# HyTruongSon/GraphFlow

Hardware: AMD Instinct MI355X
Metric: CCN-2D (SMP_omega) molecules/sec fwd+bwd (higher is better)
Workload: dtype f32 (level block products: 2xf16-split operands, 22-bit, fp32 accumulate); 1 GPU; cfg3: SMP_omega 3 levels, C=64, F=5, D=5, cap=29, batch=1024 synthetic QM9-size molecules/GPU, device-resident, fused levels; parallelism=single GPU

## Files before the change

### graphflow_amd/csrc/smp_fused.hip

```cpp
#include <algorithm>
#include <type_traits>

#include "r18_device.h"
#include "smp_internal.h"

using namespace gf::dev;

namespace gf {
namespace {

__device__ __forceinline__ f4 fold_two_tables(f4 u, f4 v) {
    f4 z;
#pragma unroll
    for (int k = 0; k < 4; ++k) {
        const auto r = __builtin_amdgcn_permlane16_swap(__float_as_uint(u[k]), __float_as_uint(v[k]), false, false);
        z[k] = xor32_sum(__uint_as_float(r[0]) + __uint_as_float(r[1]));
    }
    return z;
}

__device__ __forceinline__ f4 dpp_xor8(f4 v) {
    f4 r;
#pragma unroll
    for (int k = 0; k < 4; ++k)
        r[k] = __int_as_float(__builtin_amdgcn_update_dpp(0, __float_as_int(v[k]), 0x128 , 0xf, 0xf, true));
    return r;
}

__device__ __forceinline__ f4 dpp_ror4(f4 v) {
    f4 r;
#pragma unroll
    for (int k = 0; k < 4; ++k)
        r[k] = __int_as_float(__builtin_amdgcn_update_dpp(0, __float_as_int(v[k]), 0x124 , 0xf, 0xf, true));
    return r;
}

constexpr float kAlphaF = 0.01f;
__device__ __forceinline__ float lreluf(float z) { return z > 0.f ? z : kAlphaF * z; }

enum { T_SAB = 0, T_SBC = 1, T_T6 = 2, T_T10 = 3, T_COLS = 4 };
enum { O_LOC = 0, O_Z = 1, O_ZP = 2, O_COLS = 3 };
__constant__ int c_kperm[18] = {0, 2, 6, 5, 9, 8, 12, 11, 15, 16, 1, 3, 7, 10, 4, 13, 14, 17};

#ifndef GF_TF_DEPTH2
#define GF_TF_DEPTH2 0
#endif
#ifndef GF_TF_OCC
#define GF_TF_OCC 4
#endif
#ifndef GF_TF_WIDE
#define GF_TF_WIDE 16
#endif
#ifndef GF_TF_D2NI
#define GF_TF_D2NI 4
#endif
template <int NI, bool ALLOK, bool VEC = false, int LPC = 16>
__global__ __launch_bounds__(NI >= GF_TF_WIDE ? 2 * kThreads : kThreads, NI <= 4 ? GF_TF_OCC : 2) void smp_tables_fwd_w(
    const float *__restrict__ fprev, const float *__restrict__ rsum,
                                                             float *__restrict__ T, float *__restrict__ Vt,
                                                             float *__restrict__ scal, const long long *__restrict__ pair_src_row,
                                                             const int *__restrict__ pair_src_s, const short *__restrict__ pi,
                                                             const int4 *__restrict__ recs,
                                                             int C, int nwin,
                                                             int zeros_kept,
                                                             const unsigned char *__restrict__ rowflag,
                                                             float *__restrict__ St) {
    static_assert(!VEC || ALLOK, "the folded vector sums need every lane to have channels");
    constexpr int PPW = 64 / LPC, CWIN = 4 * LPC;
    static_assert(LPC == 16 || ((LPC == 8 || LPC == 4) && ALLOK), "eight / four lanes per position: whole 32- / 16-channel windows only");
    const int tid = threadIdx.x, lane = tid & 63;
    const int wave = __builtin_amdgcn_readfirstlane(tid >> 6);
    const int cg = lane / LPC, fl = lane % LPC;
    unsigned tile;
    {
        const unsigned nb = gridDim.x, qq = nb / 8, r = nb % 8, x = blockIdx.x % 8;
        tile = (x < r ? x * (qq + 1) : r * (qq + 1) + (x - r) * qq) + blockIdx.x / 8;
    }
    const int win = (int)(tile % nwin);
    const int4 r0 = recs[2 * (tile / nwin)], r1 = recs[2 * (tile / nwin) + 1];
    const int N = r0.y;
    const size_t rowbase = ((size_t)(unsigned)r1.y << 32) | (unsigned)r1.x, pairbase = ((size_t)(unsigned)r1.w << 32) | (unsigned)r1.z;
    const int f = win * CWIN + 4 * fl;
    const bool fok = f < C;
    const int fld = fok ? f : 0;
    constexpr bool allok = ALLOK;

    extern __shared__ __attribute__((aligned(16))) float smem[];
    constexpr int ST = PPW * NI;
    constexpr int kAbsent = 0x40000000;
    float *sR = smem;
    int4 *sRow = reinterpret_cast<int4 *>(smem + ((N + 3) & ~3));
    int *sOff = reinterpret_cast<int *>(sRow + N);
    const int nthreads = (NI >= GF_TF_WIDE ? 2 : 1) * kThreads;
    for (int i = tid; i < N; i += nthreads) {
        sR[i] = rsum[pairbase + i];
        const int sw = pair_src_s[pairbase + i];
        const unsigned long long addr = reinterpret_cast<unsigned long long>(fprev + pair_src_row[pairbase + i] * C);
        sRow[i] = make_int4((int)(unsigned)addr, (int)(unsigned)(addr >> 32), sw * sw * C * 4, sw);
    }
    for (int i = tid; i < N * ST; i += nthreads) {
        const int a = i / ST, c = i % ST;
        const int p = (c < N) ? pi[rowbase + a * N + c] : -1;
        sOff[i] = p >= 0 ? p * C * 4 : kAbsent;
    }
    unsigned char *sFlag = reinterpret_cast<unsigned char *>(sOff + N * ST);
    const bool skip_bc = zeros_kept && rowflag;
    if (skip_bc)
        for (int i = tid; i < N * N; i += nthreads) sFlag[i] = rowflag[rowbase + i];
    f4 *sAcc = reinterpret_cast<f4 *>(smem + ((((N + 3) & ~3) + 4 * N + N * ST + ((N * N + 3) >> 2) + 3) & ~3));
    const int nwv = nthreads / 64;
    f4 *wacc = sAcc + (size_t)wave * N * (2 * LPC), *wdummy = sAcc + (size_t)nwv * N * (2 * LPC) + wave * (2 * LPC);
    if constexpr (VEC)
        for (int i = lane; i < N * (2 * LPC); i += 64) wacc[i] = splat(0.f);
    __syncthreads();

    float rc[NI];
    int cc[NI];
#pragma unroll
    for (int i = 0; i < NI; ++i) {
        const int c = i * PPW + cg;
        cc[i] = (c < N) ? c : -1;
        rc[i] = (c < N && fok) ? sR[c] : 0.f;
    }
    for (int b = wave; b < N; b += nthreads / 64) {
    f4 sbc[NI], t10[NI];
#pragma unroll
    for (int i = 0; i < NI; ++i) sbc[i] = t10[i] = splat(0.f);
    f4 dgsum = splat(0.f);

    const int lane_off = fok ? fld * 4 : kAbsent;
    const int diag_off = (cg < 2) ? lane_off : kAbsent;
    auto load_row = [&](int a, f4(&v)[NI], f4 &dg) {
        const int4 ri = sRow[a];
        const int *orow = sOff + a * ST;
        const int ob = orow[b];
        int oc[NI];
#pragma unroll
        for (int i = 0; i < NI; ++i) oc[i] = orow[cg + PPW * i];
        const int od = orow[(cg == 0) ? b : a];
        const unsigned lo = __builtin_amdgcn_readfirstlane((unsigned)ri.x), hi = __builtin_amdgcn_readfirstlane((unsigned)ri.y);
        const int bytes = __builtin_amdgcn_readfirstlane(ri.z), sw = __builtin_amdgcn_readfirstlane(ri.w);
        const float *src = reinterpret_cast<const float *>(((unsigned long long)hi << 32) | lo);
        const __amdgpu_buffer_rsrc_t rs = make_rsrc(src, (size_t)(unsigned)bytes);
        const int rowoff = __builtin_amdgcn_readfirstlane(ob) * sw;
#pragma unroll
        for (int i = 0; i < NI; ++i) v[i] = buf_ld4(rs, oc[i] + lane_off, rowoff);
        dg = buf_ld4(rs, od + diag_off, rowoff);
    };

    f4 bufA[NI], bufB[NI], dA, dB;
    float *const tcol = T + (rowbase + b) * (size_t)(T_COLS * C) + f + (((lane >> 4) & 1) ? T_T6 : T_SAB) * C;
    const size_t tstep = (size_t)N * (T_COLS * C);
    unsigned present = (unsigned)__ballot(lane < N && sOff[(lane < N ? lane : 0) * ST + b] != kAbsent);
    present = __builtin_amdgcn_readfirstlane(present);
    if (allok) {
        if (!zeros_kept)
            for (unsigned z = ~present & (N >= 32 ? 0xffffffffu : ((1u << N) - 1u)); z; z &= z - 1)
                st4(tcol + (__builtin_ctz(z)) * tstep, splat(0.f));
    } else if (fok && cg < 2) {
        for (unsigned z = ~present & (N >= 32 ? 0xffffffffu : ((1u << N) - 1u)); z; z &= z - 1)
            st4(T + (rowbase + (size_t)__builtin_ctz(z) * N + b) * (size_t)(T_COLS * C) + f + (cg ? T_T6 : T_SAB) * C, splat(0.f));
    }
    auto row_step = [&](int a, int an, const f4(&cur)[NI], const f4 &dcur, f4(&nxt)[NI], f4 &dnxt, auto own_row) {
        load_row(an >= 0 ? an : a, nxt, dnxt);
        const float ra = sR[a];
        f4 sab = splat(0.f), t6 = splat(0.f);
#pragma unroll
        for (int i = 0; i < NI; ++i) {
            const f4 v = cur[i];
            sbc[i] += v;
            t10[i] += ra * v;
            sab += v;
            t6 += rc[i] * v;
        }
        if constexpr (LPC <= 8) {
            sab += dpp_xor8(sab);
            t6 += dpp_xor8(t6);
        }
        if constexpr (LPC == 4) {
            sab += dpp_ror4(sab);
            t6 += dpp_ror4(t6);
        }
        const f4 both = fold_two_tables(sab, t6);
        dgsum += dcur;
        if (allok) {
            gf_st_s<32>(reinterpret_cast<f4 *>(tcol + a * tstep), both);
            if constexpr (VEC) {
                f4 *slot = (cg == 0) ? wacc + a * (2 * LPC) + fl : wdummy + fl;
                const f4 r = slot[0] + both, d8 = slot[LPC] + dcur;
                slot[0] = r;
                slot[LPC] = d8;
            }
            if constexpr (decltype(own_row)::value) {
                if (cg == 0) st4(scal + ((pairbase + b) * 4 + 3) * (size_t)C + f, dcur);
                if (cg == 2 * (16 / LPC)) st4(scal + ((pairbase + b) * 4 + 1) * (size_t)C + f, both);
            }
        } else if (fok) {
            float *trow = T + (rowbase + (size_t)a * N + b) * (size_t)(T_COLS * C) + f;
            if (cg == 0) {
                st4(trow + T_SAB * C, both);
                if (a == b) st4(scal + ((pairbase + b) * 4 + 3) * (size_t)C + f, dcur);
            } else if (cg == 1) {
                st4(trow + T_T6 * C, both);
            } else if (cg == 2) {
                if (a == b) st4(scal + ((pairbase + b) * 4 + 1) * (size_t)C + f, both);
            }
        }
    };
    {
        auto pop = [&]() {
            if (!present) return -1;
            const int a = __builtin_ctz(present);
            present &= present - 1;
            return a;
        };
        if (ALLOK) {
            present &= ~(1u << b);
            if constexpr (GF_TF_DEPTH2 && NI <= GF_TF_D2NI) {
                f4 bufC[NI], dC;
                int a1 = pop(), a2 = pop();
                load_row(b, bufA, dA);
                load_row(a1 >= 0 ? a1 : b, bufB, dB);
                row_step(b, a2, bufA, dA, bufC, dC, std::true_type{});
                while (a1 >= 0) {
                    const int a3 = pop();
                    row_step(a1, a3, bufB, dB, bufA, dA, std::false_type{});
                    if (a2 < 0) break;
                    const int a4 = pop();
                    row_step(a2, a4, bufC, dC, bufB, dB, std::false_type{});
                    if (a3 < 0) break;
                    const int a5 = pop();
                    row_step(a3, a5, bufA, dA, bufC, dC, std::false_type{});
                    a1 = a4;
                    a2 = a5;
                }
            } else {
            int a = b, an = pop();
            load_row(a, bufA, dA);
            row_step(a, an, bufA, dA, bufB, dB, std::true_type{});
            while (an >= 0) {
                a = an;
                an = pop();
                row_step(a, an, bufB, dB, bufA, dA, std::false_type{});
                if (an < 0) break;
                a = an;
                an = pop();
                row_step(a, an, bufA, dA, bufB, dB, std::false_type{});
            }
            }
        } else {
            int a = pop();
            load_row(a, bufA, dA);
            for (;;) {
                int an = pop();
                row_step(a, an, bufA, dA, bufB, dB, std::false_type{});
                if (an < 0) break;
                a = an;
                an = pop();
                row_step(a, an, bufB, dB, bufA, dA, std::false_type{});
                if (an < 0) break;
                a = an;
            }
        }
    }
    f4 cs = splat(0.f);
#pragma unroll
    for (int i = 0; i < NI; ++i) {
        if (cc[i] >= 0) {
            cs += sbc[i];
            if (fok && (!skip_bc || (sFlag[b * N + cc[i]] & 2))) {
                float *trow = T + (rowbase + (size_t)b * N + cc[i]) * (size_t)(T_COLS * C) + f;
                gf_st_s<32>(reinterpret_cast<f4 *>(trow + T_SBC * C), sbc[i]);
                gf_st_s<32>(reinterpret_cast<f4 *>(trow + T_T10 * C), t10[i]);
            }
        }
    }
    cs = reduce_cgroups<LPC>(cs);
    const f4 dactot = shfl_xor4(dgsum, LPC);
    if (cg == 0 && fok) {
        float *v = Vt + (pairbase + b) * 4 * (size_t)C + f;
        st4(v + 1 * C, cs);
        st4(v + 3 * C, dactot);
        float *sc = scal + (pairbase + b) * 4 * (size_t)C + f;
        st4(sc + 0 * C, cs);
        st4(sc + 2 * C, dgsum);
    }
    }
    if constexpr (VEC) {
        __syncthreads();
        const int node = r0.x;
        for (int i = tid; i < N * (2 * LPC); i += nthreads) {
            const int a = i / (2 * LPC), rem = i % (2 * LPC);
            f4 v = sAcc[(size_t)a * (2 * LPC) + rem];
            for (int w = 1; w < nwv; ++w) v += sAcc[((size_t)w * N + a) * (2 * LPC) + rem];
            st4(Vt + (pairbase + a) * 4 * (size_t)C + (rem / LPC) * 2 * C + win * CWIN + 4 * (rem % LPC), v);
        }
        if (tid < 4 * LPC) {
            const int k = tid / LPC, q = tid % LPC;
            const auto one = [](int) { return 1.f; };
            st4(St + (size_t)node * 4 * C + k * C + win * CWIN + 4 * q,
                batched_sum(scal + pairbase * 4 * (size_t)C + k * C + win * CWIN + 4 * q, (size_t)4 * C, 0, N, one));
        }
    }
}

constexpr int kBigN = 64;
__global__ __launch_bounds__(256) void smp_tables_fwd_big(const float *__restrict__ fprev, const float *__restrict__ rsum, float *__restrict__ T,
                                                          float *__restrict__ Vt, float *__restrict__ scal,
                                                          const long long *__restrict__ pair_src_row, const int *__restrict__ pair_src_s,
                                                          const short *__restrict__ pi, const int *__restrict__ pair_node,
                                                          const int *__restrict__ node_s, const long long *__restrict__ node_row,
                                                          const long long *__restrict__ node_pair, long long pair0, int C, int zeros_kept,
                                                          const unsigned char *__restrict__ rowflag) {
    const long long e = pair0 + blockIdx.x;
    const int n = pair_node[e], N = node_s[n];
    const size_t rowbase = (size_t)node_row[n], pairbase = (size_t)node_pair[n];
    const int b = (int)(e - (long long)pairbase), nl = C >> 2, tid = threadIdx.x;
    extern __shared__ __attribute__((aligned(16))) float big_smem[];
    float *sBC = big_smem;
    float *sAC = sBC + (size_t)N * C;
    float *sR = sAC + (size_t)N * C;
    long long *sSrc = reinterpret_cast<long long *>(sR + ((N + 3) & ~3));
    int *sSw = reinterpret_cast<int *>(sSrc + N);
    short *sPi = reinterpret_cast<short *>(sSw + N);
    for (int i = tid; i < N; i += 256) {
        sR[i] = rsum[pairbase + i];
        sSrc[i] = pair_src_row[pairbase + i] * C;
        sSw[i] = pair_src_s[pairbase + i];
    }
    for (int i = tid; i < N * N; i += 256) sPi[i] = pi[rowbase + i];
    __syncthreads();
    const bool skip_bc = zeros_kept && rowflag;
    for (int it = tid; it < N * nl; it += 256) {
        const int c = it / nl, f = 4 * (it - c * nl);
        f4 sbc = splat(0.f), t10 = splat(0.f);
        for (int a = 0; a < N; ++a) {
            const int pb = sPi[a * N + b], pc = sPi[a * N + c];
            if (pb >= 0 && pc >= 0) {
                const f4 v = ld4(fprev + sSrc[a] + ((size_t)pb * sSw[a] + pc) * C + f);
                sbc += v;
                t10 += sR[a] * v;
            }
        }
        st4(sBC + (size_t)c * C + f, sbc);
        if (!skip_bc || (rowflag[rowbase + (size_t)b * N + c] & 2)) {
            float *trow = T + (rowbase + (size_t)b * N + c) * (size_t)(T_COLS * C) + f;
            st4(trow + T_SBC * C, sbc);
            st4(trow + T_T10 * C, t10);
        }
    }
    __syncthreads();
    f4 cs = splat(0.f);
    if (tid < nl)
        for (int c = 0; c < N; ++c) cs += ld4(sBC + (size_t)c * C + 4 * tid);
    __syncthreads();
    for (int it = tid; it < N * nl; it += 256) {
        const int a = it / nl, f = 4 * (it - a * nl);
        const int pb = sPi[a * N + b];
        f4 sab = splat(0.f), t6 = splat(0.f), dbb = splat(0.f), dac = splat(0.f);
        if (pb >= 0) {
            const float *src = fprev + sSrc[a] + (size_t)pb * sSw[a] * C + f;
            for (int c = 0; c < N; ++c) {
                const int pc = sPi[a * N + c];
                if (pc >= 0) {
                    const f4 v = ld4(src + (size_t)pc * C);
                    sab += v;
                    t6 += sR[c] * v;
                    if (c == b) dbb = v;
                    if (c == a) dac = v;
                }
            }
        }
        if (pb >= 0 || !zeros_kept) {
            float *trow = T + (rowbase + (size_t)a * N + b) * (size_t)(T_COLS * C) + f;
            st4(trow + T_SAB * C, sab);
            st4(trow + T_T6 * C, t6);
        }
        st4(sBC + (size_t)a * C + f, dbb);
        st4(sAC + (size_t)a * C + f, dac);
        if (a == b) {
            st4(scal + ((pairbase + b) * 4 + 3) * (size_t)C + f, dbb);
            st4(scal + ((pairbase + b) * 4 + 1) * (size_t)C + f, sab);
        }
    }
    __syncthreads();
    if (tid < nl) {
        const int f = 4 * tid;
        f4 dgsum = splat(0.f), dactot = splat(0.f);
        for (int a = 0; a < N; ++a) {
            dgsum += ld4(sBC + (size_t)a * C + f);
            dactot += ld4(sAC + (size_t)a * C + f);
        }
        float *v = Vt + (pairbase + b) * 4 * (size_t)C + f;
        st4(v + 1 * C, cs);
        st4(v + 3 * C, dactot);
        float *sc = scal + (pairbase + b) * 4 * (size_t)C + f;
        st4(sc + 0 * C, cs);
        st4(sc + 2 * C, dgsum);
    }
}
static size_t tables_big_lds(int N, int C) {
    return sizeof(float) * (2 * (size_t)N * C + ((N + 3) & ~3)) + sizeof(long long) * N + sizeof(int) * N + sizeof(short) * (size_t)N * N + 32;
}

__global__ __launch_bounds__(256) void smp_vectors(const float *__restrict__ T, float *__restrict__ Vt,
                                                   const float *__restrict__ scal, float *__restrict__ St,
                                                   const int *__restrict__ node_s, const long long *__restrict__ node_row,
                                                   const long long *__restrict__ node_pair, int C,
                                                   const float *__restrict__ Fdc, const long long *__restrict__ pair_src_pair,
                                                   const short *__restrict__ pi) {
    const int n = blockIdx.x;
    const int s = node_s[n], nl = C / 4;
    const size_t rowbase = (size_t)node_row[n], pairbase = (size_t)node_pair[n];
    const auto one = [](int) { return 1.f; };
    for (int i = threadIdx.x; i < s * nl; i += blockDim.x) {
        const int fl = i % nl, x = i / nl;
        const float *t = T + (rowbase + (size_t)x * s) * (size_t)(T_COLS * C) + T_SAB * C + 4 * fl;
        f4 rs = splat(0.f), d8 = splat(0.f);
        {
            const float *fd = Fdc + (size_t)pair_src_pair[pairbase + x] * 2 * C + 4 * fl;
            const short *map = pi + rowbase + (size_t)x * s;
            for (int b0 = 0; b0 < s; b0 += 8) {
                f4 v[8], u[8];
                bool ok[8];
#pragma unroll
                for (int j = 0; j < 8; ++j) {
                    const int p = (b0 + j < s) ? map[b0 + j] : -1;
                    ok[j] = p >= 0;
                    v[j] = ld4(fd + (size_t)(ok[j] ? p : 0) * 2 * C);
                    u[j] = ld4(ok[j] ? t + (size_t)(b0 + j) * (T_COLS * C) : fd);
                }
#pragma unroll
                for (int j = 0; j < 8; ++j)
                    if (ok[j]) d8 += v[j], rs += u[j];
            }
        }
        st4(Vt + (pairbase + x) * 4 * (size_t)C + 0 * C + 4 * fl, rs);
        st4(Vt + (pairbase + x) * 4 * (size_t)C + 2 * C + 4 * fl, d8);
    }
    for (int i = threadIdx.x; i < C; i += blockDim.x)
        st4(St + (size_t)n * 4 * C + 4 * i, batched_sum(scal + pairbase * 4 * (size_t)C + 4 * i, (size_t)4 * C, 0, s, one));
}

__global__ void diag_gather_fwd(const float *__restrict__ fprev, float *__restrict__ Fdc, const int *__restrict__ node_s,
                                const long long *__restrict__ node_row, const long long *__restrict__ node_pair,
                                const int *__restrict__ node_center, int C) {
    const int w = blockIdx.x;
    const int s = node_s[w], c = node_center[w], nl = C / 4;
    const float *src = fprev + (size_t)node_row[w] * C;
    float *dst = Fdc + (size_t)node_pair[w] * 2 * C;
    for (int i = threadIdx.x; i < s * nl; i += blockDim.x) {
        const int fl = i % nl, p = i / nl;
        st4(dst + (size_t)p * 2 * C + 4 * fl, ld4(src + ((size_t)p * s + p) * C + 4 * fl));
        st4(dst + (size_t)p * 2 * C + C + 4 * fl, ld4(src + ((size_t)p * s + c) * C + 4 * fl));
    }
}
// ... 433 lines not shown
    bool live[NI];
#pragma unroll
    for (int i = 0; i < NI; ++i) {
        const int c = i * PPW + cg;
        const bool ok = c < N;
        const int cx = ok ? c : 0;
        cxs[i] = cx;
        live[i] = ok && fok;
        coff[i] = cx * C + fc;
        rc[i] = L.r[cx];
        const float *t = dT + (rowbase + (size_t)b * N + cx) * (size_t)(T_COLS * C) + fc;
        yv[i] = ld4(t + T_SBC * C);
        g9[i] = ld4(t + T_T10 * C);
    }
    const int ib = b / PPW, cgb = b % PPW;
    float *dPg = dP + pbase * C + (size_t)b * N * C;
    const size_t rowStride = (size_t)N * N * C;
    for (int a = wave; a < N; a += kWaves) {
        const short *map = sPi + a * N;
        if (map[b] < 0) continue;
        float *row = dPg + a * rowStride;
        const f4 xa = ld4(sX + a * CW + 4 * fl), g5a = ld4(sG5 + a * CW + 4 * fl);
        const float ra = L.r[a];
        const int ia = a / PPW, cga = a % PPW;
        const f4 z1 = ld4(sZ1 + a * CW + 4 * fl) * ((cg == cgb) ? 1.f : 0.f);
        const f4 z2 = ld4(sZ2 + a * CW + 4 * fl) * ((cg == cga) ? 1.f : 0.f);
#pragma unroll
        for (int i = 0; i < NI; ++i) {
            f4 o = xa + yv[i] + g5a * rc[i] + g9[i] * ra;
            if (i == ib) o += z1;
            if (i == ia) o += z2;
            if (live[i] && map[cxs[i]] >= 0) st4(row + coff[i], o);
        }
    }
}

template <int LPC>
size_t tables_bwd_lds(int N) {
    constexpr int CW = 4 * LPC;
    return sizeof(float) * ((size_t)adj_lds_floats(N) + 4 * (size_t)N * CW) + sizeof(short) * (size_t)N * N + 16;
}
template <int LPC>
size_t combine_lds(int N) {
    constexpr int CW = 4 * LPC;
    return sizeof(float) * ((size_t)adj_lds_floats(N) + (size_t)kCombX * (N + 1) * CW);
}

static int node_block(const gfsmp::LevelLayout &h, int C) {
    const int smax = h.buckets.empty() ? 1 : h.buckets.back().s;
    int t = (smax * (C / 4) + 63) / 64 * 64;
    return t < 64 ? 64 : t > 256 ? 256 : t;
}

struct SizeClass {
    long long lo, hi;
    int smax, ni;
};

std::vector<SizeClass> classes_of(const gfsmp::LevelLayout &h, int ppw) {
    std::vector<SizeClass> out;
    size_t k = 0;
    for (int cls = 1; cls <= 8 && k < h.buckets.size(); cls *= 2) {
        const size_t k0 = k;
        int smax = 0;
        while (k < h.buckets.size() && h.buckets[k].s <= cls * ppw && h.buckets[k].s <= 32) smax = h.buckets[k++].s;
        if (k == k0) continue;
        SizeClass c;
        c.lo = h.node_pair[h.buckets[k0].first_node];
        c.hi = (k < h.buckets.size()) ? h.node_pair[h.buckets[k].first_node] : (long long)h.pairs;
        c.smax = smax;
        c.ni = cls;
        out.push_back(c);
    }
    return out;
}

struct BigPart {
    int n0 = 0, nodes = 0, quad0 = 0, quads = 0, smax = 0;
    long long row0 = 0, pair0 = 0, pairs = 0;
};
static BigPart big_part(const gfsmp::LevelLayout &h) {
    BigPart b;
    b.n0 = h.nNodes, b.row0 = h.rows, b.pair0 = h.pairs, b.quad0 = (int)h.quad_node.size();
    long long q = 0;
    for (const gfsmp::Bucket &bk : h.buckets) {
        if (bk.s > 32) {
            b.n0 = bk.first_node;
            break;
        }
        q += (long long)bk.count * ((bk.s + 3) / 4);
    }
    if (b.n0 < h.nNodes) {
        b.nodes = h.nNodes - b.n0;
        b.row0 = h.node_row[(size_t)b.n0], b.pair0 = h.node_pair[(size_t)b.n0];
        b.pairs = h.pairs - b.pair0;
        b.quad0 = (int)q, b.quads = (int)h.quad_node.size() - (int)q;
        b.smax = h.buckets.back().s;
    }
    return b;
}

Ragged ragged_for(const gf_smp::DevLevel &d, long long lo, int smax) {
    Ragged R = {d.pair_node, d.node_s, d.node_p, d.node_row, d.node_pair, lo, smax};
    return R;
}

static bool smp_half_window(int C) { return C % 32 == 0 && C % 64 != 0; }
static bool smp_quarter_window(int C) { return C == 16; }

static bool smp_tables_fold_vectors(const gf_smp *s) {
    return (s->cfg.nChanels & 63) == 0 || smp_half_window(s->cfg.nChanels) || smp_quarter_window(s->cfg.nChanels);
}

template <int NI>
constexpr const char *tables_fwd_name() {
    return NI == 1 ? "smpf_tables_fwd_ni1" : NI == 2 ? "smpf_tables_fwd_ni2" : NI == 4 ? "smpf_tables_fwd_ni4" : "smpf_tables_fwd_ni8";
}
template <int NI, int LPC>
gf_status launch_tables_fwd_wn(gf_smp *s, int l, const SizeClass &c) {
    gf_ctx *ctx = s->ctx;
    const gf_smp::DevLevel &d = s->lv[l];
    const gfsmp::LevelLayout &h = s->lay.level[l];
    const int C = s->cfg.nChanels, nwin = C / (4 * LPC);
    constexpr int PPW = 64 / LPC;
    const int n_lo = h.pair_node[(size_t)c.lo], n_hi = (c.hi < (long long)h.pairs) ? h.pair_node[(size_t)c.hi] : h.nNodes;
    if (n_hi <= n_lo) return GF_OK;
    const size_t lds = sizeof(float) * ((c.smax + 3) & ~3) + 16 * (size_t)c.smax + sizeof(int) * (size_t)c.smax * PPW * NI + 16 +
                       (size_t)c.smax * c.smax + 16;
    const int nwv = kThreads / 64;
    const size_t lds_v = ((lds + 15) & ~(size_t)15) + 16 + (size_t)nwv * ((size_t)c.smax * (32 * LPC) + 32 * LPC);
    gf_status st = opt_in_lds(ctx, smp_tables_fwd_w<NI, true, true, LPC>, lds_v);
    if (st != GF_OK) return st;
    const int flags = d.t_zeros ? 1 : 0;
    GF_LAUNCH(ctx, tables_fwd_name<NI>(), (smp_tables_fwd_w<NI, true, true, LPC>), dim3((unsigned)((n_hi - n_lo) * nwin)), dim3(kThreads), lds_v,
              s->lv[l - 1].f, d.rsum, d.Q, d.Vt, d.scal, d.pair_src_row, d.pair_src_s, d.pi, d.tf_recs + 2 * (size_t)n_lo, C, nwin,
              flags, flags ? d.rowflag : (const unsigned char *)nullptr, d.St);
    return GF_OK;
}

template <int NI>
gf_status launch_tables_fwd_w(gf_smp *s, int l, const SizeClass &c) {
    gf_ctx *ctx = s->ctx;
    const gf_smp::DevLevel &d = s->lv[l];
    const gfsmp::LevelLayout &h = s->lay.level[l];
    const int C = s->cfg.nChanels, nwin = (C + 63) / 64;
    const int n_lo = h.pair_node[(size_t)c.lo], n_hi = (c.hi < (long long)h.pairs) ? h.pair_node[(size_t)c.hi] : h.nNodes;
    if (n_hi <= n_lo) return GF_OK;
    const size_t lds = sizeof(float) * ((c.smax + 3) & ~3) + 16 * (size_t)c.smax + sizeof(int) * (size_t)c.smax * 4 * NI + 16 +
                       (size_t)c.smax * c.smax + 16;
    const int flags = ((d.t_zeros && (C & 63) == 0) ? 1 : 0);
    if (smp_tables_fold_vectors(s)) {
        const int nwv = (NI >= GF_TF_WIDE ? 2 : 1) * kThreads / 64;
        const size_t lds_v = ((lds + 15) & ~(size_t)15) + 16 + (size_t)nwv * ((size_t)c.smax * 512 + 512);
        gf_status st = opt_in_lds(ctx, smp_tables_fwd_w<NI, true, true>, lds_v);
        if (st != GF_OK) return st;
        GF_LAUNCH(ctx, tables_fwd_name<NI>(), (smp_tables_fwd_w<NI, true, true>), dim3((unsigned)((n_hi - n_lo) * nwin)), dim3((NI >= GF_TF_WIDE ? 2 : 1) * kThreads), lds_v,
                  s->lv[l - 1].f, d.rsum, d.Q, d.Vt, d.scal, d.pair_src_row, d.pair_src_s, d.pi, d.tf_recs + 2 * (size_t)n_lo, C, nwin,
                  flags, flags ? d.rowflag : (const unsigned char *)nullptr, d.St);
    } else
        GF_LAUNCH(ctx, tables_fwd_name<NI>(), (smp_tables_fwd_w<NI, false>), dim3((unsigned)((n_hi - n_lo) * nwin)), dim3((NI >= GF_TF_WIDE ? 2 : 1) * kThreads), lds,
                  s->lv[l - 1].f, d.rsum, d.Q, d.Vt, d.scal, d.pair_src_row, d.pair_src_s, d.pi, d.tf_recs + 2 * (size_t)n_lo, C, nwin,
                  flags, (const unsigned char *)nullptr, (float *)nullptr);
    return GF_OK;
}

template <int NI>
gf_status launch_tables_bwd(gf_smp *s, int l, const SizeClass &c, const float *dT) {
    gf_ctx *ctx = s->ctx;
    const gf_smp::DevLevel &d = s->lv[l];
    const int C = s->cfg.nChanels, nwin = (C + 63) / 64;
    const size_t lds = tables_bwd_lds<16>(c.smax);
    gf_status st = opt_in_lds(ctx, smp_tables_bwd<16, NI>, lds);
    if (st != GF_OK) return st;
    GF_LAUNCH(ctx, "smpf_tables_bwd", (smp_tables_bwd<16, NI>), dim3((unsigned)((c.hi - c.lo) * nwin)), dim3(kThreads), lds, dT,
              d.dVt, d.dSt, d.adj, s->P, d.pi, ragged_for(d, c.lo, c.smax), C, nwin);
    return GF_OK;
}


constexpr int kGatherMaxS = 64;

struct GatherTables {
    const int4 *hdr;
    const int4 *qrec;
};

__global__ __launch_bounds__(64) void build_gather_records(const int *__restrict__ prev_s, const long long *__restrict__ cons_ptr,
                                     const long long *__restrict__ cons_qbase, const int *__restrict__ cons_s,
                                     const int *__restrict__ cons_a, const long long *__restrict__ cons_row,
                                     const long long *__restrict__ cons_pair, const int *__restrict__ pair_node,
                                     const long long *__restrict__ cons_inv_off, const short *__restrict__ inv,
                                     const float *__restrict__ rsum, int ldt_bytes, int4 *__restrict__ hdr, int4 *__restrict__ qrec) {
    const int w = blockIdx.x, sw = prev_s[w];
    const int pad = gfsmp::gather_pad(sw);
    const long long c0 = cons_ptr[w], c1 = cons_ptr[w + 1], qb = cons_qbase[w];
    for (long long ce = c0 + threadIdx.x; ce < c1; ce += blockDim.x) {
        const long long row = cons_row[ce], pe = cons_pair[ce], pb = pe - cons_a[ce];
        hdr[2 * ce] = make_int4(cons_s[ce], cons_a[ce], (int)(unsigned)(row & 0xffffffffll), (int)(row >> 32));
        hdr[2 * ce + 1] = make_int4((int)(unsigned)(pb & 0xffffffffll), (int)(pb >> 32), pair_node[pe], __float_as_int(rsum[pe]));
    }
    const long long n = (c1 - c0) * pad;
    for (long long i = threadIdx.x; i < n; i += blockDim.x) {
        const long long ce = c0 + i / pad;
        const int q = (int)(i % pad);
        const long long pe = cons_pair[ce], pb = pe - cons_a[ce];
        const int c = q < sw ? (int)inv[cons_inv_off[ce] + q] : -1;
        int cfirst = 0;
        for (int k = 0; k < sw; ++k) {
            const int ck = (int)inv[cons_inv_off[ce] + k];
            if (ck >= 0) {
                cfirst = ck;
                break;
            }
        }
        const float ra = rsum[pe], rho = c >= 0 ? rsum[pb + c] : 0.f, m = c >= 0 ? 1.f : 0.f;
        qrec[qb + i] = make_int4((c >= 0 ? c : cfirst) * ldt_bytes, __float_as_int(rho), __float_as_int(m), __float_as_int(m * ra));
    }
}

typedef int si4 __attribute__((ext_vector_type(4)));
__device__ __forceinline__ si4 s_load4(const int4 *p) {
    si4 r;
    asm volatile("s_load_dwordx4 %0, %1, 0x0" : "=s"(r) : "s"(p));
    return r;
}
__device__ __forceinline__ void s_wait2(si4 &a, si4 &b) { asm volatile("s_waitcnt lgkmcnt(0)" : "+s"(a), "+s"(b)); }
template <int N>
__device__ __forceinline__ void s_wait(si4 (&r)[N]) {
    if constexpr (N == 1) asm volatile("s_waitcnt lgkmcnt(0)" : "+s"(r[0]));
    else if constexpr (N == 2) asm volatile("s_waitcnt lgkmcnt(0)" : "+s"(r[0]), "+s"(r[1]));
    else if constexpr (N == 4) asm volatile("s_waitcnt lgkmcnt(0)" : "+s"(r[0]), "+s"(r[1]), "+s"(r[2]), "+s"(r[3]));
    else if constexpr (N == 5) asm volatile("s_waitcnt lgkmcnt(0)" : "+s"(r[0]), "+s"(r[1]), "+s"(r[2]), "+s"(r[3]), "+s"(r[4]));
    else if constexpr (N == 6)
        asm volatile("s_waitcnt lgkmcnt(0)" : "+s"(r[0]), "+s"(r[1]), "+s"(r[2]), "+s"(r[3]), "+s"(r[4]), "+s"(r[5]));
    else {
        static_assert(N == 8, "batch sizes of the gather");
        asm volatile("s_waitcnt lgkmcnt(0)"
                     : "+s"(r[0]), "+s"(r[1]), "+s"(r[2]), "+s"(r[3]), "+s"(r[4]), "+s"(r[5]), "+s"(r[6]), "+s"(r[7]));
    }
}

__device__ __forceinline__ f4 gbuf_ld4_once(__amdgpu_buffer_rsrc_t r, int voff_bytes) {
    return __builtin_bit_cast(f4, __builtin_amdgcn_raw_buffer_load_b128(r, voff_bytes, 0, (GF_NT_SITES & 128) ? 2 : 0));
}
constexpr int kOor = 0x40000000;

#define GF_GATHER_PARAMS                                                                                                          \
    const float *__restrict__ dT, const float *__restrict__ dVt, const float *__restrict__ dSt, float *__restrict__ dfprev,            \
        const float *__restrict__ dFdc, const int *__restrict__ prev_s, const long long *__restrict__ prev_row,                      \
        const long long *__restrict__ prev_pair, const int *__restrict__ prev_center, const long long *__restrict__ cons_ptr,        \
        const long long *__restrict__ cons_inv_off, const long long *__restrict__ cons_qbase, const short *__restrict__ inv,         \
        GatherTables G, int C
#define GF_GATHER_ARGS dT, dVt, dSt, dfprev, dFdc, prev_s, prev_row, prev_pair, prev_center, cons_ptr, cons_inv_off, cons_qbase, inv, G, C

template <int SWP, int QB, int RS = SWP>
__device__ __forceinline__ void gather_source(GF_GATHER_PARAMS, int w, int chunk, int qoff = 0) {
    static_assert(SWP % QB == 0, "whole batches");
    const int sw = prev_s[w], cw = prev_center[w];
    const int nl = C >> 2, items = sw * nl;
    const long long c0 = cons_ptr[w], c1 = cons_ptr[w + 1];
    const int C4 = C * 4, ldtb = T_COLS * C4;
    float *dst = dfprev + prev_row[w] * C;
    const float *dfd = dFdc + (size_t)prev_pair[w] * 2 * C;
    const long long ioff0 = c0 < c1 ? cons_inv_off[c0] : 0;
    const int4 *qr0 = G.qrec + cons_qbase[w];
    {
        const int it = chunk * 64 + (int)(threadIdx.x & 63);
        const bool live = it < items;
        const int p = live ? it / nl : 0, f4b = 16 * (live ? it % nl : 0);
        f4 acc[SWP], accd = splat(0.f), accc = splat(0.f);
#pragma unroll
        for (int q = 0; q < SWP; ++q) acc[q] = splat(0.f);
        if (live) {
            accd = ld4(dfd + (size_t)p * 2 * C + (f4b >> 2));
            accc = ld4(dfd + (size_t)p * 2 * C + C + (f4b >> 2));
        }
        if (c0 < c1) {
            si4 h0 = s_load4(G.hdr + 2 * c0), h1 = s_load4(G.hdr + 2 * c0 + 1);
            s_wait2(h0, h1);
            int b = inv[ioff0 + p];
            b = live ? b : -1;
            for (long long ce = c0; ce < c1; ++ce) {
                const long long cn = ce + 1 < c1 ? ce + 1 : ce;
                si4 n0 = s_load4(G.hdr + 2 * cn), n1 = s_load4(G.hdr + 2 * cn + 1);
                int bn = inv[ioff0 + (cn - c0) * sw + p];
                bn = live ? bn : -1;
                const int s = h0.x, a = h0.y;
                const long long urow = ((long long)h0.w << 32) | (unsigned)h0.z, upb = ((long long)h1.y << 32) | (unsigned)h1.x;
                const int unode = h1.z;
                const __amdgpu_buffer_rsrc_t rT = make_rsrc(dT + (size_t)urow * (T_COLS * C), (size_t)s * s * ldtb);
                const __amdgpu_buffer_rsrc_t rV = make_rsrc(dVt + (size_t)upb * 4 * C, (size_t)s * 4 * C4);
                const __amdgpu_buffer_rsrc_t rS = make_rsrc(dSt + (size_t)unode * 4 * C, (size_t)4 * C4);
                const bool has = b >= 0;
                const int tab = has ? (a * s + b) * ldtb + f4b : kOor;
                const int va = has ? a * 4 * C4 + f4b : kOor, vb = has ? b * 4 * C4 + f4b : kOor;
                const int vs = has ? f4b : kOor, vd = (has && p == cw) ? f4b : kOor;
                const int tb = has ? b * s * ldtb + f4b : kOor;
                const f4 l0 = gbuf_ld4_once(rT, tab + T_SAB * C4), g5 = gbuf_ld4_once(rT, tab + T_T6 * C4);
                const f4 l1 = buf_ld4(rV, va, 0), l4 = buf_ld4(rV, va + 2 * C4, 0);
                const f4 l2 = buf_ld4(rV, vb + C4, 0), z2 = buf_ld4(rV, vb + 3 * C4, 0);
                const f4 l3 = buf_ld4(rS, vs, 0), l5 = buf_ld4(rS, vs + 2 * C4, 0);
                const f4 l6 = buf_ld4(rS, vd + C4, 0), l7 = buf_ld4(rS, vd + 3 * C4, 0);
                const int4 *qr = qr0 + (ce - c0) * RS + qoff;
                f4 x = splat(0.f);
#pragma unroll
                for (int q0 = 0; q0 < SWP; q0 += QB) {
// ... 700 lines not shown
```

Before: 164,100 molecules/s.

## Dispatch forward table kernel to exact-width NI instantiation per node size

Moves the forward table-building body into a device function and adds a multi-width kernel that picks, per node, the template instantiation whose position count NI is just large enough for that node's size, through a wave-uniform switch. A size class no longer pays for the worst-case NI registers and loop trips on smaller nodes. It also rebuilds the per-slot column index inside the store loop instead of keeping it in a register array, to ease register pressure. In exchange the kernel grows in code size and may need more registers, since one kernel holds several inlined bodies. It is on by default for NI 4 and 8 when vector folding is enabled, and an environment variable turns it off.

```diff
diff --git a/graphflow_amd/csrc/smp_fused.hip b/graphflow_amd/csrc/smp_fused.hip
--- a/graphflow_amd/csrc/smp_fused.hip
+++ b/graphflow_amd/csrc/smp_fused.hip
@@ -54,30 +54,21 @@
 #ifndef GF_TF_D2NI
 #define GF_TF_D2NI 4
 #endif
-template <int NI, bool ALLOK, bool VEC = false, int LPC = 16>
-__global__ __launch_bounds__(NI >= GF_TF_WIDE ? 2 * kThreads : kThreads, NI <= 4 ? GF_TF_OCC : 2) void smp_tables_fwd_w(
-    const float *__restrict__ fprev, const float *__restrict__ rsum,
-                                                             float *__restrict__ T, float *__restrict__ Vt,
-                                                             float *__restrict__ scal, const long long *__restrict__ pair_src_row,
-                                                             const int *__restrict__ pair_src_s, const short *__restrict__ pi,
-                                                             const int4 *__restrict__ recs,
-                                                             int C, int nwin,
-                                                             int zeros_kept,
-                                                             const unsigned char *__restrict__ rowflag,
-                                                             float *__restrict__ St) {
+template <int NI, bool ALLOK, bool VEC, int LPC>
+__device__ __forceinline__ void tables_fwd_node(const float *__restrict__ fprev, const float *__restrict__ rsum, float *__restrict__ T,
+                                                float *__restrict__ Vt, float *__restrict__ scal, const long long *__restrict__ pair_src_row,
+                                                const int *__restrict__ pair_src_s, const short *__restrict__ pi,
+                                                const int4 r0, const int4 r1,
+                                                const int win, int C,
+                                                int zeros_kept,
+                                                const unsigned char *__restrict__ rowflag,
+                                                float *__restrict__ St) {
     static_assert(!VEC || ALLOK, "the folded vector sums need every lane to have channels");
     constexpr int PPW = 64 / LPC, CWIN = 4 * LPC;
     static_assert(LPC == 16 || ((LPC == 8 || LPC == 4) && ALLOK), "eight / four lanes per position: whole 32- / 16-channel windows only");
     const int tid = threadIdx.x, lane = tid & 63;
     const int wave = __builtin_amdgcn_readfirstlane(tid >> 6);
     const int cg = lane / LPC, fl = lane % LPC;
-    unsigned tile;
-    {
-        const unsigned nb = gridDim.x, qq = nb / 8, r = nb % 8, x = blockIdx.x % 8;
-        tile = (x < r ? x * (qq + 1) : r * (qq + 1) + (x - r) * qq) + blockIdx.x / 8;
-    }
-    const int win = (int)(tile % nwin);
-    const int4 r0 = recs[2 * (tile / nwin)], r1 = recs[2 * (tile / nwin) + 1];
     const int N = r0.y;
     const size_t rowbase = ((size_t)(unsigned)r1.y << 32) | (unsigned)r1.x, pairbase = ((size_t)(unsigned)r1.w << 32) | (unsigned)r1.z;
     const int f = win * CWIN + 4 * fl;
@@ -115,11 +106,9 @@
     __syncthreads();
 
     float rc[NI];
-    int cc[NI];
 #pragma unroll
     for (int i = 0; i < NI; ++i) {
         const int c = i * PPW + cg;
-        cc[i] = (c < N) ? c : -1;
         rc[i] = (c < N && fok) ? sR[c] : 0.f;
     }
     for (int b = wave; b < N; b += nthreads / 64) {
@@ -264,12 +253,15 @@
         }
     }
     f4 cs = splat(0.f);
+    int cg_b = cg;
+    asm volatile("" : "+v"(cg_b));
 #pragma unroll
     for (int i = 0; i < NI; ++i) {
-        if (cc[i] >= 0) {
+        const int c = i * PPW + cg_b;
+        if (c < N) {
             cs += sbc[i];
-            if (fok && (!skip_bc || (sFlag[b * N + cc[i]] & 2))) {
-                float *trow = T + (rowbase + (size_t)b * N + cc[i]) * (size_t)(T_COLS * C) + f;
+            if (fok && (!skip_bc || (sFlag[b * N + c] & 2))) {
+                float *trow = T + (rowbase + (size_t)b * N + c) * (size_t)(T_COLS * C) + f;
                 gf_st_s<32>(reinterpret_cast<f4 *>(trow + T_SBC * C), sbc[i]);
                 gf_st_s<32>(reinterpret_cast<f4 *>(trow + T_T10 * C), t10[i]);
             }
@@ -302,6 +294,44 @@
                 batched_sum(scal + pairbase * 4 * (size_t)C + k * C + win * CWIN + 4 * q, (size_t)4 * C, 0, N, one));
         }
     }
+}
+
+__device__ __forceinline__ unsigned tables_fwd_tile() {
+    const unsigned nb = gridDim.x, qq = nb / 8, r = nb % 8, x = blockIdx.x % 8;
+    return (x < r ? x * (qq + 1) : r * (qq + 1) + (x - r) * qq) + blockIdx.x / 8;
+}
+
+template <int NI, bool ALLOK, bool VEC = false, int LPC = 16>
+__global__ __launch_bounds__(NI >= GF_TF_WIDE ? 2 * kThreads : kThreads, NI <= 4 ? GF_TF_OCC : 2) void smp_tables_fwd_w(
+    const float *__restrict__ fprev, const float *__restrict__ rsum, float *__restrict__ T, float *__restrict__ Vt, float *__restrict__ scal,
+    const long long *__restrict__ pair_src_row, const int *__restrict__ pair_src_s, const short *__restrict__ pi,
+    const int4 *__restrict__ recs,
+    int C, int nwin, int zeros_kept, const unsigned char *__restrict__ rowflag, float *__restrict__ St) {
+    const unsigned tile = tables_fwd_tile();
+    const int4 r0 = recs[2 * (tile / nwin)], r1 = recs[2 * (tile / nwin) + 1];
+    tables_fwd_node<NI, ALLOK, VEC, LPC>(fprev, rsum, T, Vt, scal, pair_src_row, pair_src_s, pi, r0, r1, (int)(tile % nwin), C, zeros_kept, rowflag, St);
+}
+
+template <int NI0, int NI1, int OCC>
+__global__ __launch_bounds__(kThreads, OCC) void smp_tables_fwd_m(
+    const float *__restrict__ fprev, const float *__restrict__ rsum, float *__restrict__ T, float *__restrict__ Vt, float *__restrict__ scal,
+    const long long *__restrict__ pair_src_row, const int *__restrict__ pair_src_s, const short *__restrict__ pi,
+    const int4 *__restrict__ recs,
+    int C, int nwin, int zeros_kept, const unsigned char *__restrict__ rowflag, float *__restrict__ St) {
+    static_assert(GF_TF_WIDE > 8 && NI0 >= 1 && NI1 <= 8, "the exact-width entries run four waves per node, at most 32 positions");
+    const unsigned tile = tables_fwd_tile();
+    const int4 r0 = recs[2 * (tile / nwin)], r1 = recs[2 * (tile / nwin) + 1];
+    const int win = (int)(tile % nwin);
+#define GF_TF_CASE(K)                                                                                                                        \
+    case K:                                                                                                                                  \
+        if constexpr (K >= NI0 && K <= NI1)                                                                                                  \
+            tables_fwd_node<K, true, true, 16>(fprev, rsum, T, Vt, scal, pair_src_row, pair_src_s, pi, r0, r1, win, C, zeros_kept, rowflag, St); \
+        break;
+    switch (__builtin_amdgcn_readfirstlane((r0.y + 3) >> 2)) {
+        GF_TF_CASE(1) GF_TF_CASE(2) GF_TF_CASE(3) GF_TF_CASE(4) GF_TF_CASE(5) GF_TF_CASE(6) GF_TF_CASE(7) GF_TF_CASE(8)
+        default: break;
+    }
+#undef GF_TF_CASE
 }
 
 constexpr int kBigN = 64;
@@ -1041,6 +1071,16 @@
     if (smp_tables_fold_vectors(s)) {
         const int nwv = (NI >= GF_TF_WIDE ? 2 : 1) * kThreads / 64;
         const size_t lds_v = ((lds + 15) & ~(size_t)15) + 16 + (size_t)nwv * ((size_t)c.smax * 512 + 512);
+        if constexpr (NI == 4 || NI == 8) {
+            if (!env_is("GF_SMP_TF_CLASSES", '0')) {
+                gf_status st = opt_in_lds(ctx, smp_tables_fwd_m<NI / 2 + 1, NI, (NI == 4 ? GF_TF_OCC : 2)>, lds_v);
+                if (st != GF_OK) return st;
+                GF_LAUNCH(ctx, tables_fwd_name<NI>(), (smp_tables_fwd_m<NI / 2 + 1, NI, (NI == 4 ? GF_TF_OCC : 2)>), dim3((unsigned)((n_hi - n_lo) * nwin)),
+                          dim3(kThreads), lds_v, s->lv[l - 1].f, d.rsum, d.Q, d.Vt, d.scal, d.pair_src_row, d.pair_src_s, d.pi,
+                          d.tf_recs + 2 * (size_t)n_lo, C, nwin, flags, flags ? d.rowflag : (const unsigned char *)nullptr, d.St);
+                return GF_OK;
+            }
+        }
         gf_status st = opt_in_lds(ctx, smp_tables_fwd_w<NI, true, true>, lds_v);
         if (st != GF_OK) return st;
         GF_LAUNCH(ctx, tables_fwd_name<NI>(), (smp_tables_fwd_w<NI, true, true>), dim3((unsigned)((n_hi - n_lo) * nwin)), dim3((NI >= GF_TF_WIDE ? 2 : 1) * kThreads), lds_v,
```

Result: no change. 165,600 molecules/s, median of 6 (+0.9%).
